# thuml/HashGAN

Hardware: AMD Instinct MI355X
Metric: queries/sec (mAP@R of Q queries vs N-code database, Hamming ranking) (higher is better)
Workload: dtype fp4 (E2M1 0/+-1) x fp4 -> f32 exact distances; u32 xor+popcount elsewhere; f64 AP; 1 GPU; C2: Q=10000 N=1000000 b=64 R=5000 C=10, planted codes; parallelism=1 GPU

## Files before the change

### hashgan_amd/csrc/hg_core.hip

```cpp
#include "hg_ctx.hpp"
#include "hg_host_pack.hpp"

#include <exception>
#include <map>
#include <mutex>
#include <thread>
#include <unistd.h>

thread_local std::string g_err;

int fail(int code, const char* fmt, ...) {
    char buf[512];
    va_list ap;
    va_start(ap, fmt);
    vsnprintf(buf, sizeof buf, fmt, ap);
    va_end(ap);
    g_err = buf;
    return code;
}

const char* const kKernelNames[KI_COUNT] = {"k_hist", "k_hist_reduce", "k_plan", "k_seg_counts", "k_seg_layout", "k_guess",
                                            "k_select", "k_rank_hist", "k_order", "k_rank_fused", "k_match", "k_ap", "k_merge", "k_pack",
                                            "k_real_sample", "k_real_guess", "k_real_select", "k_radix_pass", "k_real_finish", "k_select_mx", "k_rank_cnt", "rccl_allgather", "step_gpu_span", "k_real_rescore"};
void build_shape(int n, ApShape& sh) {
// ... 553 lines not shown
    if (Q < 1 || !host_x || !host_labels) return fail(HG_ERR_ARG, "hg_set_queries_f32: need Q >= 1 and data");
    if (Q > 0x7FFFFFC0ll) return fail(HG_ERR_ARG, "hg_set_queries_f32: Q too large");
    const i64 old_q = c->Q;
    const bool had_q = (c->stage & ST_Q) != 0;
    c->Q = Q;
    if (c->opt.host_pack) {
        const int saved_bpad = c->bpad;
        HG_TRY(pack_on_host(c, host_x, host_labels, Q, c->qc, c->qlab, c->qf, c->dbf_resident ? 1 : 0, &c->qf_resident,
                            bad_codes, bad_labels, c->census_q));
        if (!c->qf_resident) c->bpad = saved_bpad;
    } else {
        HG_TRY(pack_on_device(c, host_x, host_labels, Q, c->qc, c->qlab, c->qf, bad_codes, bad_labels, c->census_q));
        c->qf_resident = true;
    }
    c->stage = ST_DB | ST_Q;
    c->qx_valid = false;
    queries_replaced(c, old_q, had_q);
    return HG_OK;
}

int hg_get_packed(hg_ctx* c, int which, uint32_t* host_codes, uint64_t* host_labels) {
    HG_TRY(need(c, which ? (ST_DB | ST_Q) : ST_DB, "hg_get_packed", "hg_set_database / hg_set_queries"));
    const i64 n = which ? c->Q : c->N;
    DevBuf& cd = which ? c->qc : c->db;
    DevBuf& lb = which ? c->qlab : c->dblab;
    if (host_codes) HG_HIP(hipMemcpyAsync(host_codes, cd.p, (size_t)n * c->NW * 4, hipMemcpyDeviceToHost, c->stream));
    if (host_labels) HG_HIP(hipMemcpyAsync(host_labels, lb.p, (size_t)n * c->LW * 8, hipMemcpyDeviceToHost, c->stream));
    return c->sync();
}

int hg_set_queries(hg_ctx* c, const uint64_t* codes, const uint64_t* labels, int64_t Q) {
// ... 18 lines not shown
    memcpy((char*)qs.pin + cb, labels, lb);
    HG_TRY(c->qc.reserve((size_t)Q * c->NW * 4 + 64 * 4));
    HG_TRY(c->qlab.reserve(lb));
    if (cb + lb <= ((size_t)4 << 20)) {
        const i64 nc = (i64)Q * c->NW, nl = (i64)Q * c->LW * 2;
        hipLaunchKernelGGL(k_copy_in, dim3(grid_for(nc + nl)), dim3(256), 0, c->stream, (const u32*)qs.pin, c->qc.as<u32>(), nc, 2 * W, c->NW,
                           (const u32*)((const char*)qs.pin + cb), c->qlab.as<u32>(), nl);
        HG_TRY(c->check_launch("k_copy_in"));
    } else {
        HG_TRY(upload_codes(c, c->qc, (const uint64_t*)qs.pin, Q, W, c->NW));
        HG_HIP(hipMemcpyAsync(c->qlab.p, (const char*)qs.pin + cb, lb, hipMemcpyHostToDevice, c->stream));
    }
    HG_HIP(hipEventRecord(qs.ev, c->stream));
    qs.used = true;
    c->stage = ST_DB | ST_Q;
    c->qx_valid = false;
    c->qf_resident = false;
    queries_replaced(c, old_q, had_q);
    return HG_OK;
}

extern "C++" int do_match(hg_ctx* c) {
    const Geo& g = c->geo;
    const i64 nKB = (g.R + 255) / 256;
    const i64 blocks = nKB * g.Q;
    if (blocks > 0x7FFFFFFFll) return fail(HG_ERR_ARG, "hg_match: Q*R too large for one launch");
    c->t_begin(KI_MATCH);
    hipLaunchKernelGGL(k_match, dim3((unsigned)blocks), dim3(256), 0, c->stream, c->out_idx.as<u32>(),
                       c->dblab.as<u64>(), c->qlab.as<u64>(), c->mbits.as<u64>(), c->RW, (int)nKB, g);
    c->t_end();
    HG_TRY(c->check_launch("k_match"));
// ... 372 lines not shown
        *value = kind == 0 ? g_host_ns[ph].load() / 1000 : kind == 1 ? g_host_calls[ph].load() : g_host_max_ns[ph].load() / 1000;
    }
    else if (!strcmp(key, "graph_replays")) *value = c->graph_replays;
    else if (!strcmp(key, "cut_beyond_planes")) {
        u32 v = 0;
        if (c->beyond.p) {
            HG_HIP(hipMemcpyAsync(&v, c->beyond.p, 4, hipMemcpyDeviceToHost, c->stream));
            HG_TRY(c->sync());
        }
        *value = v;
    }
    else if (!strcmp(key, "map_async_steps")) *value = c->map_async_steps;
    else if (!strcmp(key, "map_async_redone")) *value = c->map_async_redone;
    else if (!strcmp(key, "map_overlapped_steps")) *value = c->map_overlapped;
    else if (!strcmp(key, "segments")) *value = c->geo.S;
    else if (!strcmp(key, "records_kept")) {
        const Geo& g = c->geo;
        *value = -1;
        if (c->optimistic && c->sl_cnt.p && c->sl_cnt.cap >= (size_t)g.S * g.Qpad * 4) {
            HG_TRY(c->use());
            HG_TRY(c->sync());
            std::vector<u32> h((size_t)g.S * g.Qpad);
            HG_HIP(hipMemcpy(h.data(), c->sl_cnt.p, h.size() * 4, hipMemcpyDeviceToHost));
            i64 total = 0;
            for (int s = 0; s < g.S; ++s) for (int q = 0; q < g.Q; ++q) total += h[(size_t)s * g.Qpad + q];
            *value = total;
        }
    }
    else return fail(HG_ERR_ARG, "hg_get_stat: unknown key '%s'", key);
    return HG_OK;
// ... 45 lines not shown
```

### hashgan_amd/csrc/hg_ctx.hpp

```cpp
#pragma once
#include "hg_kernels.hpp"
#pragma GCC visibility push(default)
#include "../../include/hashgan_amd.h"
#pragma GCC visibility pop

#include <rccl/rccl.h>
#include <atomic>
#include <chrono>
#include <cmath>
#include <cstdarg>
#include <cstdio>
#include <cstdlib>
#include <cstring>
#include <string>
#include <utility>
#include <vector>

using namespace hg;

extern thread_local std::string g_err;
int fail(int code, const char* fmt, ...);

#define HG_HIP(expr)                                                                         \
    do {                                                                                     \
// ... 276 lines not shown
    bool crowd_probed = false;
    i64 crowd_x100 = 0;
    i64 cap_boost = 1;
    i64 real_cap_boost = 1;
    bool leftovers_expected = false;
    bool last_leftovers_inline = false;

    bool want_lists = true;
    i64 bet_runs = 0, bet_fallbacks = 0, bet_requeried = 0;
    i64 rank_leftovers = 0;
    int bet_consecutive_fail = 0;
    int shard_bet_fail = 0;
    hg_ctx* sub = nullptr;
    bool is_sub = false;

    bool dbx_valid = false, qx_valid = false, dbx8_valid = false, dbx3_valid = false, dbx4_valid = false;
    bool hist_pairs = false;
    i64 bet_rebets = 0;
    bool verdict_pending = false, verdict_known = false;
    int verdict_flag = 0;
    void* pin = nullptr;
    size_t pin_cap = 0;
    struct MapSlot {
        void* pin = nullptr; size_t cap = 0; hipEvent_t ev = nullptr;
        bool async = false;
        bool inline_ok = false;
        i64 R = 0, Q = 0;
        unsigned long long q_gen = 0, db_gen = 0;
        std::vector<double> ap; std::vector<int64_t> rel;
    } mslot[2];
    int ms_head = 0, ms_n = 0;
// ... 30 lines not shown
    void* hpk = nullptr;
    size_t hpk_cap = 0;
    bool dbf_resident = false, qf_resident = false;
    RealState real;
    bool real_lists = false;
    i64 shapes_for_R = -1;
    i64 recip_for_R = -1;

    ncclComm_t comm = nullptr;
    int comm_rank = 0, comm_world = 1;

    DevBuf db, dblab, qc, qlab;
    DevBuf dbf, qf;
    DevBuf dbx, qx;
    DevBuf dbx8;
    DevBuf dbx3;
    DevBuf dbx4;
    DevBuf dbfx;
    DevBuf dbfb, xmax2;
    DevBuf shapes, ap_recip;
    DevBuf seglt, segtie;
    DevBuf mbits2;
    DevBuf part;
    DevBuf obuf[2];
    DevBuf beyond;
    DevBuf stage_in, badcnt;
    DevBuf flist;
    DevBuf dbytes;
    DevBuf samp, thr, sortA, sortB, scores, gtab;
    DevBuf sampx;
    DevBuf cntq;
    DevBuf krows;
    DevBuf thr2;
    DevBuf hist2;
    DevBuf gathered[4], scratch[4], comm_tmp, gath_idx, gath_dist;

    template <class F> void for_each_buf(F&& f) {
        for (DevBuf* d : {&db, &dblab, &qc, &qlab, &dbf, &qf}) f(*d, BUF_TABLE);
        for (DevBuf* d : {&dbx, &qx, &dbx8, &dbx3, &dbx4, &dbfx, &dbfb, &xmax2, &shapes, &ap_recip}) f(*d, BUF_DERIVED);
        for (DevBuf* d : {&seglt, &segtie, &mbits2, &part, &obuf[0], &obuf[1], &beyond, &stage_in, &badcnt, &flist, &dbytes, &samp, &thr,
                          &sortA, &sortB, &scores, &gtab, &sampx, &cntq, &krows, &thr2, &hist2, &comm_tmp, &gath_idx, &gath_dist})
            f(*d, BUF_WORK);
        for (DevBuf& d : gathered) f(d, BUF_WORK);
        for (DevBuf& d : scratch) f(d, BUF_WORK);
        for_each_step_buf(f);
        ws_b.for_each_step_buf(f);
    }
    void forget_derived() {
        dbx_valid = qx_valid = dbx8_valid = dbx3_valid = dbx4_valid = dbfx_valid = dbfb_valid = false;
        shapes_for_R = recip_for_R = -1;
        outblk_q = ws_b.outblk_q = -1;
    }

    struct StepGraph {
        hipGraph_t graph = nullptr;
        hipGraphExec_t exec = nullptr;
        unsigned long long epoch = 0, cfg = 0, seen_epoch = 0, seen_cfg = 0;
        i64 R = -1, seen_R = -1;
        int timing = -1, seen_timing = -1;
        StepState left;
        std::vector<Pending> evs;
    } sg;
    unsigned long long cfg_epoch = 1;
    bool capturing = false;
// ... 103 lines not shown
int do_ap_range(hg_ctx* c, i64 q0, i64 nq, const u32* only = nullptr);
inline int do_ap(hg_ctx* c) { return do_ap_range(c, 0, c->geo.Q); }
int ensure_out_block(hg_ctx* c);
int read_plan_flag(hg_ctx* c, int* flag);
int launch_min_topr(hg_ctx* c, const u32* idx_all, const u8* dist_all, i64 n, int G);
hg_ctx* requery_child(hg_ctx* c, i64 nF);
int stage_ap_download(hg_ctx* c, void* dst = nullptr);
int wait_verdict(hg_ctx* c, bool staged, int* flag);
void make_geometry(hg_ctx* c);
Geo hist_geometry(const hg_ctx* c);
int set_R(hg_ctx* c, int64_t R, int G, int rank);
int launch_hist(hg_ctx* c);
int launch_select_valu(hg_ctx* c, int lw, bool optimistic);
int launch_select_dense(hg_ctx* c, int lw);
int ensure_mx_images(hg_ctx* c, bool need_db);
int launch_hist_mx(hg_ctx* c);
int launch_select_mx(hg_ctx* c, int lw, const int* cut);
int launch_select_mx3(hg_ctx* c, int lw, const int* cut);
int launch_select_mx4(hg_ctx* c, int lw, const int* cut);
int preload_valu(); int preload_mx(); int preload_mx1(); int preload_real(); int preload_seq();
void comm_release(hg_ctx* c);

#define HG_DISPATCH_NW(fn, c, ...)                              \
    switch ((c)->NW) {                                          \
        case 1: return fn<1>(c, ##__VA_ARGS__);                 \
        case 2: return fn<2>(c, ##__VA_ARGS__);                 \
        case 3: return fn<3>(c, ##__VA_ARGS__);                 \
        case 4: return fn<4>(c, ##__VA_ARGS__);                 \
        case 5: return fn<5>(c, ##__VA_ARGS__);                 \
        case 6: return fn<6>(c, ##__VA_ARGS__);                 \
// ... 5 lines not shown
```

### hashgan_amd/csrc/hg_hist_i8.hpp

```cpp
#pragma once
#include "hg_kernels.hpp"
#include "hg_hist_mx.hpp"

namespace hg {

typedef int i32x16 __attribute__((ext_vector_type(16)));
typedef __attribute__((address_space(3))) u32 lds_u32;

__device__ __forceinline__ void lds_add_at(const u32 addr, const u32 inc) {
#if defined(__HIP_DEVICE_COMPILE__)
    __hip_atomic_fetch_add((lds_u32*)addr, inc, __ATOMIC_RELAXED, __HIP_MEMORY_SCOPE_WORKGROUP);
#else
    (void)addr; (void)inc;
#endif
}

__device__ __forceinline__ uint4 bits16_to_bytes(const u32 bits, const u32 one, const u32 zero) {
    u32 w[4];
#pragma unroll
    for (int d = 0; d < 4; ++d) {
        u32 v = 0;
#pragma unroll
        for (int i = 0; i < 4; ++i) v |= (((bits >> (4 * d + i)) & 1u) ? one : zero) << (8 * i);
        w[d] = v;
    }
    return uint4{w[0], w[1], w[2], w[3]};
}

static __global__ __launch_bounds__(256) void k_expand_db_i8(const u32* __restrict__ db, uint4* __restrict__ img, i64 N, i64 n16, int NW) {
    const i64 i = (i64)blockIdx.x * 256 + threadIdx.x;
    if (i >= n16 * NW * 2) return;
    const i64 row = i / (NW * 2);
    const int c = (int)(i - row * NW * 2), m = c >> 1, hh = c & 1;
    const u32 word = row < N ? db[row * NW + m] : 0u;
    img[(((row >> 4) * NW + m) * 2 + hh) * 16 + (row & 15)] = bits16_to_bytes((word >> (16 * hh)) & 0xFFFFu, 8u, 0u);
}

constexpr int hist_i8_cols(bool pack16) { return pack16 ? 1 : 2; }

template <int NW, bool PACK16>
__global__ __launch_bounds__(256) __attribute__((amdgpu_waves_per_eu(4, 4)))
void k_hist_i8(const u32* __restrict__ qc, const u8* __restrict__ dbx8, u32* __restrict__ hist, const Geo g) {
    extern __shared__ __attribute__((aligned(16))) u32 hlds[];
    constexpr int QT = 2, WQ = 32 * QT;
    const int lb = logical_block(g.nBlk);
    if (lb < 0) return;
    const int lane = threadIdx.x & 63;
    const int wave = __builtin_amdgcn_readfirstlane(threadIdx.x >> 6);
    const int nQB = g.nQT;
    const int sp = lb / nQB, qb = lb - sp * nQB;
    const int h = lane >> 5, j = lane & 31;
    const int NB = g.NB, b = g.NB - 1;
    const i64 lo0 = (i64)(2 * sp) * g.L, lo1 = lo0 + g.L;
    const i64 len0 = (lo0 + g.L < g.N ? g.L : g.N - lo0);
    const i64 len1 = lo1 >= g.N ? 0 : (lo1 + g.L < g.N ? g.L : g.N - lo1);
    const i64 mylen = h ? len1 : len0;
    const i64 ntile = ((len0 > len1 ? len0 : len1) + 15) / 16;
    const i64 NG = (g.N + 15) >> 4;
    const int stride = g.hist_stride;

    constexpr int NCOL = hist_i8_cols(PACK16);
    u32* col = hlds + wave * NCOL * NB * 32;
    for (int i = lane; i < NCOL * NB * 32; i += 64) col[i] = 0u;

    const int q0w = (qb * WPB + wave) * WQ;
    i32x4 bq[QT][NW];
    i32x16 biasv[QT];
    u32 inc[QT];
#pragma unroll
    for (int t = 0; t < QT; ++t) {
        const int q = q0w + t * 32 + j;
        int pop = 0;
#pragma unroll
        for (int m = 0; m < NW; ++m) {
            const u32 word = q < g.Q ? qc[(i64)q * NW + m] : 0u;
            pop += __builtin_popcount(word);
            const int first = 32 * m + 16 * h;
            const u32 valid = b - first >= 16 ? 0xFFFFu : (b - first <= 0 ? 0u : (1u << (b - first)) - 1u);
            const u32 bits = (word >> (16 * h)) & 0xFFFFu;
            const uint4 neg = bits16_to_bytes(bits & valid, 0xF0u, 0u);
            const uint4 pos = bits16_to_bytes(~bits & valid, 0x10u, 0u);
            bq[t][m] = i32x4{(int)(neg.x | pos.x), (int)(neg.y | pos.y), (int)(neg.z | pos.z), (int)(neg.w | pos.w)};
        }
        u32* c0 = col + (PACK16 ? 0 : t * NB * 32) + j;
        const int base = (int)(u32)(size_t)(lds_u32*)c0 + 128 * pop;
#pragma unroll
        for (int r = 0; r < 16; ++r) biasv[t][r] = base;
        inc[t] = PACK16 ? (t ? 65536u : 1u) : 1u;
    }
    wave_lds_sync();

    const int ah = (j >> 2) & 1;
    const int ar = (j & 3) + 4 * (j >> 3);
    const i64 ag0 = (ah ? lo1 : lo0) >> 4;
    auto chunk = [&](const i64 T, const int m) -> i32x4 {
        i64 G = ag0 + T;
        G = G < NG ? G : NG - 1;
        return *(const i32x4*)(dbx8 + ((((G * NW + m) * 2 + h) * 16 + ar) * 16));
// ... 20 lines not shown
                for (int r = 0; r < 16; ++r)
                    lds_add_at((u32)acc[r], inc[t]);
            } else {
#pragma unroll
                for (int r = 0; r < 16; ++r)
                    if ((i64)r < left) lds_add_at((u32)acc[r], inc[t]);
            }
        }
#pragma unroll
        for (int m = 0; m < NW; ++m) av[m] = an[m];
    }
    wave_lds_sync();
    const int q = q0w + lane;
    if (q < g.Qpad) {
        u32* __restrict__ out = hist + (i64)sp * NB * g.Qpad + q;
        const int dn = g.hcap > 0 && g.hcap < NB ? g.hcap : NB;
        for (int d = 0; d < dn; ++d) {
            const u32 v = PACK16 ? (col[d * 32 + j] >> (16 * h)) & 0xFFFFu : col[(h * NB + d) * 32 + j];
            out[(i64)d * g.Qpad] = v;
        }
    }
}

}
```

### hashgan_amd/csrc/hg_packed_drain.hpp

```cpp
#pragma once
#include "hg_select_mx.hpp"

namespace hg {

constexpr int PK_QCAP = 128;
constexpr int PK_RING = 16;

__device__ __forceinline__ u32 pk_and_or(const u32 x, const u32 k, const u32 y) {
    u32 d;
    asm("v_and_or_b32 %0, %1, %2, %3" : "=v"(d) : "v"(x), "n"(k), "v"(y));
    return d;
}

struct PackedLds {
    int a, abuf;
    int cl, clbuf, labels;
    int qcodes, qlabels;
    int queue;
    int rings;
    int total;
};
template <class P> __host__ __device__ inline PackedLds packed_lds_layout(int NW, int LW) {
    PackedLds l;
    const int WS = P::ws(LW), WROWS = WS * P::ROWS;
// ... 236 lines not shown
                const u8* ring = rings + ring_index(t) * PK_RING;
                *(u64*)(slice(t) + min(f, cap - 8u)) = *(const u64*)(ring + (f & 8u));
            }
        }
    }
};

template <int LW, class P>
struct PackedBlock {
    int sp, qb;
    int h, j;
    int s;
    bool seg_ok;
    i64 lo0, lo1, len0, len1;
    i64 mylen, minlen;
    i64 nwin;
    i64 NG;

    __device__ __forceinline__ PackedBlock(const int lb, const int lane, const Geo& g) {
        constexpr int WROWS = P::ws(LW) * P::ROWS;
        const int nQB = g.nQT;
        sp = lb / nQB;
        qb = lb - sp * nQB;
        h = lane >> 5; j = lane & 31;
        s = 2 * sp + h;
        seg_ok = s < g.S;
        lo0 = (i64)(2 * sp) * g.L; lo1 = lo0 + g.L;
        len0 = (lo0 + g.L < g.N ? g.L : g.N - lo0);
        len1 = lo1 >= g.N ? 0 : (lo1 + g.L < g.N ? g.L : g.N - lo1);
        mylen = h ? len1 : len0;
        minlen = len0 < len1 ? len0 : len1;
        nwin = ((len0 > len1 ? len0 : len1) + WROWS - 1) / WROWS;
        NG = (g.N + P::ROWS - 1) / P::ROWS;
    }
};

}
```

### hashgan_amd/csrc/hg_pairs_mx.hip

```cpp
#include "hg_ctx.hpp"
#include "hg_mx_drain.hpp"
#include "hg_select_mx.hpp"
#include "hg_select_mx3.hpp"
#include "hg_select_mx4.hpp"
#include "hg_hist_mx.hpp"
#include "hg_hist_i8.hpp"

int ensure_mx_images(hg_ctx* c, const bool need_db) {
    const int NW = c->NW, NM = (NW + 1) / 2;
    if (need_db && !c->dbx_valid) {
        const i64 n16 = (c->N + 15) / 16 * 16;
        HG_TRY(c->dbx.reserve((size_t)(n16 > 0 ? n16 : 16) * NM * 32));
        const i64 items = n16 * 2 * NM;
        c->t_begin(KI_PACK);
        if (items) hipLaunchKernelGGL(k_expand_db, dim3(grid_for(items)), dim3(256), 0, c->stream, c->db.as<u32>(),
                                      c->dbx.as<uint4>(), (i64)c->N, n16, NW, NM);
        c->t_end();
        HG_TRY(c->check_launch("k_expand_db"));
        c->dbx_valid = true;
    }
    if (!c->qx_valid) {
        const i64 qpad = ((i64)c->Q + 511) / 512 * 512;
        HG_TRY(c->qx.reserve((size_t)qpad * NM * 32));
        const i64 items = qpad * 2 * NM;
        c->t_begin(KI_PACK);
        hipLaunchKernelGGL(k_expand_queries, dim3(grid_for(items)), dim3(256), 0, c->stream, c->qc.as<u32>(), c->qx.as<uint4>(),
                           (i64)c->Q, qpad, NW, NM);
        c->t_end();
        HG_TRY(c->check_launch("k_expand_queries"));
        c->qx_valid = true;
    }
    return HG_OK;
}


namespace {
template <int NW> int launch_hist_mx_t(hg_ctx* c) {
    HG_TRY(ensure_mx_images(c, true));
    Geo g = c->geo;
    const int nSP = (g.S + 1) / 2;
    const int nQB = (g.Q + 255) / 256;
    g.nQT = nQB;
    g.nUnits = (i64)nSP * nQB;
    g.wpb = WPB;
    g.nBlk = (int)g.nUnits;
    const i64 tiles_per_half = ((g.L + 15) / 16 + g.hist_stride - 1) / g.hist_stride;
    const i64 visited_per_pair = 2 * tiles_per_half * 16;
    const bool pack16 = visited_per_pair < 65536;
    const size_t lds = (size_t)WPB * (pack16 ? 1 : 2) * g.NB * 32 * 4;
// ... 50 lines not shown
template <int NW, int LW> int launch_select_mx4_t(hg_ctx* c, const int* cut) {
    return launch_select_packed<M4Pack>(c, cut, NW, LW, c->dbx4, c->dbx4_valid, k_expand_db4, "k_expand_db4", &k_select_mx4<NW, LW>, "k_select_mx4");
}

template <int NW> int launch_hist_i8_t(hg_ctx* c) {
    if (!c->dbx8_valid) {
        const i64 n16 = (c->N + 15) / 16 * 16;
        HG_TRY(c->dbx8.reserve((size_t)n16 * NW * 32));
        c->t_begin(KI_PACK);
        hipLaunchKernelGGL(k_expand_db_i8, dim3(grid_for(n16 * NW * 2)), dim3(256), 0, c->stream, c->db.as<u32>(), c->dbx8.as<uint4>(),
                           (i64)c->N, n16, NW);
        c->t_end();
        HG_TRY(c->check_launch("k_expand_db_i8"));
        c->dbx8_valid = true;
    }
    Geo g = c->geo;
    const int nSP = (g.S + 1) / 2;
    const int nQB = (g.Q + 255) / 256;
    g.nQT = nQB;
    g.nUnits = (i64)nSP * nQB;
    g.wpb = WPB;
    g.nBlk = (int)g.nUnits;
    const i64 tiles_per_half = ((g.L + 15) / 16 + g.hist_stride - 1) / g.hist_stride;
    const bool pack16 = 2 * tiles_per_half * 16 < 65536;
    const size_t lds = (size_t)WPB * hist_i8_cols(pack16) * g.NB * 32 * 4;
    c->t_begin(KI_HIST);
    if (pack16) {
        if (lds > 64 * 1024)
            HG_HIP(hipFuncSetAttribute(reinterpret_cast<const void*>(&k_hist_i8<NW, true>), hipFuncAttributeMaxDynamicSharedMemorySize, (int)lds));
        hipLaunchKernelGGL((k_hist_i8<NW, true>), dim3(padded_grid(g.nBlk)), dim3(256), lds, c->stream, c->qc.as<u32>(), c->dbx8.as<u8>(),
                           c->hist.as<u32>(), g);
    } else {
        if (lds > 64 * 1024)
            HG_HIP(hipFuncSetAttribute(reinterpret_cast<const void*>(&k_hist_i8<NW, false>), hipFuncAttributeMaxDynamicSharedMemorySize, (int)lds));
        hipLaunchKernelGGL((k_hist_i8<NW, false>), dim3(padded_grid(g.nBlk)), dim3(256), lds, c->stream, c->qc.as<u32>(), c->dbx8.as<u8>(),
                           c->hist.as<u32>(), g);
    }
    c->t_end();
    return c->check_launch("k_hist_i8");
}
}

int launch_hist_mx(hg_ctx* c) {
    if (c->opt.hist_mfma == 2 && c->NW <= 4) {
        switch (c->NW) {
            case 1: return launch_hist_i8_t<1>(c);
            case 2: return launch_hist_i8_t<2>(c);
            case 3: return launch_hist_i8_t<3>(c);
            default: return launch_hist_i8_t<4>(c);
        }
    }
// ... 22 lines not shown
```

### hashgan_amd/csrc/hg_select_mx3.hpp

```cpp
#pragma once
#include "hg_packed_drain.hpp"

namespace hg {

constexpr int M3_QT = 2;
constexpr int M3_ROWS = 48;
#ifndef HG_M3_WS
#define HG_M3_WS 4
#endif
__host__ __device__ constexpr int m3_ws(int LW) { return LW <= 1 ? HG_M3_WS : 2; }
constexpr int M3_WS_MAX = HG_M3_WS > 2 ? HG_M3_WS : 2;
#ifndef HG_M3_WPB
#define HG_M3_WPB 8
#endif
#ifndef HG_M3_FLUSH
#define HG_M3_FLUSH 4
#endif
#ifndef HG_M3_ILV
#define HG_M3_ILV 8
#endif
constexpr int M3_WPB = HG_M3_WPB;

__host__ __device__ constexpr int m3_row(int f, int r) { return r < 7 ? 7 * f + r : r < 14 ? 21 + 7 * f + (r - 7) : 42 + 2 * f + (r - 14); }
__host__ __device__ constexpr int m3_shift(int r) { return r < 7 ? r % 3 : r < 14 ? (r - 7) % 3 : r - 14; }
// ... 82 lines not shown
    constexpr int QT = M3_QT, WQ = 32 * QT;
    constexpr int CB = NW * 4, LB = LW * 8;
    constexpr int M3_WS = m3_ws(LW), M3_WROWS = M3_WS * M3_ROWS;
    const PackedLds L = packed_lds_layout<M3Pack>(NW, LW);

    const int lb = logical_block(g.nBlk);
    if (lb < 0) return;
    const int lane = threadIdx.x & 63;
    const int wave = __builtin_amdgcn_readfirstlane(threadIdx.x >> 6);
    const PackedBlock<LW, M3Pack> blk(lb, lane, g);
    const int h = blk.h, j = blk.j, s = blk.s;
    const bool seg_ok = blk.seg_ok;
    const i64 lo0 = blk.lo0, lo1 = blk.lo1, nwin = blk.nwin, NG = blk.NG;

    const int q0w = (blk.qb * M3_WPB + wave) * WQ;
    {
        u32* qcl = (u32*)(mxlds + L.qcodes + wave * WQ * CB);
        for (int e = lane; e < WQ * NW; e += 64) {
            const i64 q = q0w + e / NW;
            qcl[e] = q < g.Q ? qc[q * NW + (e % NW)] : 0u;
        }
        u64* qll = (u64*)(mxlds + L.qlabels + wave * WQ * LB);
        for (int e = lane; e < WQ * LW; e += 64) {
            const i64 q = q0w + e / LW;
            qll[e] = q < g.Q ? qlab[q * LW + (e % LW)] : 0ull;
        }
    }
    i32x4 bq[QT];
    f32x16 cv[QT];
    u32 K[QT][3];
// ... 80 lines not shown
#undef HG_U
        asm volatile("" : "+v"(w[0]), "+v"(w[1]), "+v"(w[2]));
    };

    int clsel = 0;
    if (nwin > 0) stage_window(0, 0, 0);
    for (i64 win = 0; win < nwin; ++win) {
        const int abuf = (int)(win & 1);
        const int clnext = clsel == 2 ? 0 : clsel + 1;
        asm volatile("s_waitcnt vmcnt(0)" ::: "memory");
        __syncthreads();
        if (win + 1 < nwin) stage_window(win + 1, abuf ^ 1, clnext);
        const u8* sa = mxlds + L.a + abuf * L.abuf;
#pragma unroll
        for (int st = 0; st < M3_WS; ++st) {
            i32x4 af[3];
#pragma unroll
            for (int f = 0; f < 3; ++f) af[f] = *(const i32x4*)(sa + ((st * 3 + f) * 64 + lane) * 16);
            f32x16 acc[QT];
#pragma unroll
            for (int t = 0; t < QT; ++t) acc[t] = cv[t];
            u32 w[QT][3];
#if HG_M3_ILV
#pragma unroll
            for (int t = 0; t < QT; ++t) {
                const i32x8 B = {bq[t].x, bq[t].y, bq[t].z, bq[t].w, 0, 0, 0, 0};
#pragma unroll
                for (int f = 0; f < 3; ++f) {
                    const i32x8 A = {af[f].x, af[f].y, af[f].z, af[f].w, 0, 0, 0, 0};
                    acc[t] = f == 0 ? __builtin_amdgcn_mfma_scale_f32_32x32x64_f8f6f4(A, B, acc[t], 4, 4, 0, scale_a, 0, scale_b)
// ... 25 lines not shown
            for (int t = 0; t < QT; ++t) harvest(acc[t], t, w[t]);
#endif
            const i64 base_row = win * M3_WROWS + st * M3_ROWS;
            if (blk.minlen - base_row < M3_ROWS) {
                const i64 left = blk.mylen - base_row;
                const int la = left < 0 ? 0 : left > 21 ? 21 : (int)left, lb2 = left < 21 ? 0 : left > 42 ? 21 : (int)left - 21;
                const u32 ka = ((1u << la) - 1u) << 6, kb = ((1u << lb2) - 1u) << 6;
                u32 kc = 0;
                for (int c = 0; c < 6; ++c) if (42 + c < left) kc |= 1u << (6 + 7 * (c >> 1) + (c & 1));
#pragma unroll
                for (int t = 0; t < QT; ++t) { w[t][0] &= ka; w[t][1] &= kb; w[t][2] &= kc; }
            }
            if (!(kProbes && (a.probe & 2))) dr.push(w, st, (u32)clsel);
            __builtin_amdgcn_sched_barrier(0);
        }
        if (!(kProbes && (a.probe & 2))) dr.end_window(((win + 1) * M3_WS) % M3Pack::FLUSH == 0);
        clsel = clnext;
    }
    dr.finish();

#pragma unroll
    for (int t = 0; t < QT; ++t) {
        const int q = q0w + t * 32 + j;
        if (seg_ok && q < g.Qpad) {
            const bool live = q < g.Q;
            a.sl_cnt[(i64)s * g.Qpad + q] = live ? (dr.cnt[t] < a.cap ? dr.cnt[t] : a.cap) : 0u;
            if ((dr.cnt[t] > a.cap || far[t]) && live) a.fail[q] = 1u;
        }
    }
}

}
```

### hashgan_amd/csrc/hg_select_mx4.hpp

```cpp
#pragma once
#include "hg_packed_drain.hpp"

namespace hg {

constexpr int M4_QT = 2;
constexpr int M4_ROWS = 32;
#ifndef HG_M4_WS
#define HG_M4_WS 2
#endif
constexpr int M4_WS = HG_M4_WS;
constexpr int M4_WPB = 8;
constexpr int M4_NM = 2;

__host__ __device__ constexpr int m4_row(int f, int r) { return 16 * (r >> 3) + 8 * f + (r & 7); }
__host__ __device__ constexpr int m4_shift(int r) { return r & 7; }
__host__ __device__ inline void m4_place(int rho, int& f, int& r) {
    f = (rho >> 3) & 1;
    r = 8 * (rho >> 4) + (rho & 7);
}

static __global__ __launch_bounds__(256) void k_expand_db4(const u32* __restrict__ db, uint4* __restrict__ dbx, i64 N, i64 n32, int NW) {
    const i64 i = (i64)blockIdx.x * 256 + threadIdx.x;
    if (i >= n32 * 4) return;
    const i64 row = i >> 2;
// ... 48 lines not shown
    constexpr int CB = NW * 4, LB = LW * 8;
    constexpr int WROWS = M4_WS * M4_ROWS;
    constexpr int NM = M4_NM;
    const PackedLds L = packed_lds_layout<M4Pack>(NW, LW);

    const int lb = logical_block(g.nBlk);
    if (lb < 0) return;
    const int lane = threadIdx.x & 63;
    const int wave = __builtin_amdgcn_readfirstlane(threadIdx.x >> 6);
    const PackedBlock<LW, M4Pack> blk(lb, lane, g);
    const int h = blk.h, j = blk.j, s = blk.s;
    const bool seg_ok = blk.seg_ok;
    const i64 lo0 = blk.lo0, lo1 = blk.lo1, nwin = blk.nwin, NG = blk.NG;

    const int q0w = (blk.qb * M4_WPB + wave) * WQ;
    {
        u32* qcl = (u32*)(mxlds + L.qcodes + wave * WQ * CB);
        for (int e = lane; e < WQ * NW; e += 64) {
            const i64 q = q0w + e / NW;
            qcl[e] = q < g.Q ? qc[q * NW + (e % NW)] : 0u;
        }
        u64* qll = (u64*)(mxlds + L.qlabels + wave * WQ * LB);
        for (int e = lane; e < WQ * LW; e += 64) {
            const i64 q = q0w + e / LW;
            qll[e] = q < g.Q ? qlab[q * LW + (e % LW)] : 0ull;
        }
    }
    i32x4 bq[QT][NM];
    f32x16 cv[QT];
    u32 alive[QT];
// ... 83 lines not shown
#undef HG_U
        asm volatile("" : "+v"(w[0]), "+v"(w[1]));
    };

    int clsel = 0;
    if (nwin > 0) stage_window(0, 0, 0);
    for (i64 win = 0; win < nwin; ++win) {
        const int abuf = (int)(win & 1);
        const int clnext = clsel == 2 ? 0 : clsel + 1;
        asm volatile("s_waitcnt vmcnt(0)" ::: "memory");
        __syncthreads();
        if (win + 1 < nwin) stage_window(win + 1, abuf ^ 1, clnext);
        const u8* sa = mxlds + L.a + abuf * L.abuf;
#pragma unroll
        for (int st = 0; st < M4_WS; ++st) {
            u32 w[QT][2];
#if HG_M4_SEQ
#pragma unroll
            for (int t = 0; t < QT; ++t) {
                f32x16 acc = cv[t];
#pragma unroll
                for (int f = 0; f < 2; ++f) {
#pragma unroll
                    for (int m = 0; m < NM; ++m) {
                        const i32x4 af = *(const i32x4*)(sa + (((st * 2 + f) * NM + m) * 64 + lane) * 16);
                        const i32x8 A = {af.x, af.y, af.z, af.w, 0, 0, 0, 0};
                        const i32x8 B = {bq[t][m].x, bq[t][m].y, bq[t][m].z, bq[t][m].w, 0, 0, 0, 0};
                        acc = f == 0 ? __builtin_amdgcn_mfma_scale_f32_32x32x64_f8f6f4(A, B, acc, 4, 4, 0, scale_a, 0, scale_b)
                                     : __builtin_amdgcn_mfma_scale_f32_32x32x64_f8f6f4(A, B, acc, 4, 4, 1, scale_a, 0, scale_b);
                    }
// ... 20 lines not shown
            }
#pragma unroll
            for (int t = 0; t < QT; ++t) harvest(acc[t], t, w[t]);
#endif
            const i64 base_row = win * WROWS + st * M4_ROWS;
            if (blk.minlen - base_row < M4_ROWS) {
                const i64 left = blk.mylen - base_row;
                const int la = left < 0 ? 0 : left > 16 ? 16 : (int)left, lb2 = left < 16 ? 0 : left > 32 ? 16 : (int)left - 16;
                const u32 ka = ((1u << la) - 1u) << 7, kb = ((1u << lb2) - 1u) << 7;
#pragma unroll
                for (int t = 0; t < QT; ++t) { w[t][0] &= ka; w[t][1] &= kb; }
            }
            if (!(kProbes && (a.probe & 2))) dr.push(w, st, (u32)clsel);
            __builtin_amdgcn_sched_barrier(0);
        }
        if (!(kProbes && (a.probe & 2))) dr.end_window(((win + 1) * M4_WS) % M4Pack::FLUSH == 0);
        clsel = clnext;
    }
    dr.finish();

#pragma unroll
    for (int t = 0; t < QT; ++t) {
        const int q = q0w + t * 32 + j;
        if (seg_ok && q < g.Qpad) {
            const bool live = q < g.Q;
            a.sl_cnt[(i64)s * g.Qpad + q] = live ? (dr.cnt[t] < a.cap ? dr.cnt[t] : a.cap) : 0u;
            if ((dr.cnt[t] > a.cap || far[t]) && live) a.fail[q] = 1u;
        }
    }
}

}
```

### hashgan_amd/csrc/hg_seq.hip

```cpp
#include "hg_ctx.hpp"
#include <chrono>
#include "hg_select_mx.hpp"
#include "hg_select_mx3.hpp"
#include "hg_select_mx4.hpp"
#include "hg_hist_mx.hpp"
#include "hg_rank_cnt.hpp"
#include "hg_rank_lean.hpp"
#include "hg_rank_dense.hpp"

constexpr i64 SAMPLE_RATIO = 2;

void make_geometry(hg_ctx* c) {
    Geo& g = c->geo;
    g.Q = (int)c->Q;
    g.nQT = (int)((c->Q + 63) / 64);
    g.Qpad = g.nQT * 64;
    g.NW = c->NW; g.NB = c->NB; g.LW = c->LW;
    g.N = c->N; g.R = c->R; g.idx_base = c->idx_base;
    i64 S = (c->opt.target_units + g.nQT - 1) / g.nQT;
    if (S > c->opt.max_segments) S = c->opt.max_segments;
    const i64 maxS = (c->N + c->opt.min_segment - 1) / c->opt.min_segment;
    if (S > maxS) S = maxS;
    if (S < 1) S = 1;
    i64 L = (c->N + S - 1) / S;
// ... 1328 lines not shown
    c->last_leftovers_inline = false;
    HG_TRY(run_oneshot(c, R, false, true));
    HG_TRY(hg_get_ap(c, host_ap, host_rel));
    if (c->optimistic && c->bet_fallbacks + c->bet_requeried + c->bet_rebets == fails0 && (c->rank_leftovers == left0 || c->last_leftovers_inline) && !c->is_sub) {
        c->map_warm_cfg = c->cfg_epoch; c->map_warm_epoch = g_alloc_epoch; c->map_warm_R = R;
        if (c->opt.step_streams >= 2 && c->own_stream && !c->stream_b) HG_TRY(stream_create(c->device, &c->stream_b));
    } else {
        c->map_warm_R = -1;
    }
    return HG_OK;
}

static int prepare_shared(hg_ctx* c, int64_t R, bool* enqueued) {
    *enqueued = false;
    if (c->opt.select_mfma && !c->qx_valid) { HG_TRY(ensure_mx_images(c, false)); *enqueued = true; }
    const bool recip = c->opt.ap_recip && R <= (1ll << 20);
    if (c->shapes_for_R != R || (recip && c->recip_for_R != R)) {
        HG_TRY(set_R(c, R, 1, 0));
        bool use_recip = false;
        HG_TRY(ensure_ap_tables(c, &use_recip));
        *enqueued = true;
    }
    return HG_OK;
}

static int enqueue_bet_on_b(hg_ctx* c, hg_ctx::MapSlot& m, int64_t R, int stride, bool tail_fork) {
    if (!c->stream_b) HG_TRY(stream_create(c->device, &c->stream_b));
    if (!c->ev_pre) HG_HIP(hipEventCreateWithFlags(&c->ev_pre, hipEventDisableTiming));
    if (!c->ev_fork) HG_HIP(hipEventCreateWithFlags(&c->ev_fork, hipEventDisableTiming));
    if (tail_fork || !c->pre_valid) {
// ... 113 lines not shown
```

Before: 12.20 million queries/s.

## Precompute int8 query image for histogram and skip idle waves in MFMA select

Adds a cached int8 query image with per-query popcounts, built once per query set, so k_hist_i8 loads query fragments instead of expanding bits per block. The histogram LDS clear is limited to the capped distance range. The mx3/mx4 select kernels skip waves whose queries lie entirely past Q and stop stepping past the real segment length, avoiding padded MFMA work. This adds a derived buffer and its validity tracking, and makes the image build part of prepare_shared.

Result: no change. 12.30 million queries/s, median of 6 (+0.8%).

```diff
diff --git a/hashgan_amd/csrc/hg_core.hip b/hashgan_amd/csrc/hg_core.hip
--- a/hashgan_amd/csrc/hg_core.hip
+++ b/hashgan_amd/csrc/hg_core.hip
@@ -591,7 +591,7 @@
         c->qf_resident = true;
     }
     c->stage = ST_DB | ST_Q;
-    c->qx_valid = false;
+    c->qx_valid = c->qx8_valid = false;
     queries_replaced(c, old_q, had_q);
     return HG_OK;
 }
@@ -640,7 +640,7 @@
     HG_HIP(hipEventRecord(qs.ev, c->stream));
     qs.used = true;
     c->stage = ST_DB | ST_Q;
-    c->qx_valid = false;
+    c->qx_valid = c->qx8_valid = false;
     c->qf_resident = false;
     queries_replaced(c, old_q, had_q);
     return HG_OK;
@@ -1043,6 +1043,7 @@
     else if (!strcmp(key, "map_async_redone")) *value = c->map_async_redone;
     else if (!strcmp(key, "map_overlapped_steps")) *value = c->map_overlapped;
     else if (!strcmp(key, "segments")) *value = c->geo.S;
+    else if (!strcmp(key, "segment_rows")) *value = c->geo.L;
     else if (!strcmp(key, "records_kept")) {
         const Geo& g = c->geo;
         *value = -1;
diff --git a/hashgan_amd/csrc/hg_ctx.hpp b/hashgan_amd/csrc/hg_ctx.hpp
--- a/hashgan_amd/csrc/hg_ctx.hpp
+++ b/hashgan_amd/csrc/hg_ctx.hpp
@@ -314,7 +314,7 @@
     hg_ctx* sub = nullptr;
     bool is_sub = false;
 
-    bool dbx_valid = false, qx_valid = false, dbx8_valid = false, dbx3_valid = false, dbx4_valid = false;
+    bool dbx_valid = false, qx_valid = false, qx8_valid = false, dbx8_valid = false, dbx3_valid = false, dbx4_valid = false;
     bool hist_pairs = false;
     i64 bet_rebets = 0;
     bool verdict_pending = false, verdict_known = false;
@@ -375,6 +375,7 @@
     DevBuf dbf, qf;
     DevBuf dbx, qx;
     DevBuf dbx8;
+    DevBuf qx8;
     DevBuf dbx3;
     DevBuf dbx4;
     DevBuf dbfx;
@@ -398,7 +399,7 @@
 
     template <class F> void for_each_buf(F&& f) {
         for (DevBuf* d : {&db, &dblab, &qc, &qlab, &dbf, &qf}) f(*d, BUF_TABLE);
-        for (DevBuf* d : {&dbx, &qx, &dbx8, &dbx3, &dbx4, &dbfx, &dbfb, &xmax2, &shapes, &ap_recip}) f(*d, BUF_DERIVED);
+        for (DevBuf* d : {&dbx, &qx, &dbx8, &qx8, &dbx3, &dbx4, &dbfx, &dbfb, &xmax2, &shapes, &ap_recip}) f(*d, BUF_DERIVED);
         for (DevBuf* d : {&seglt, &segtie, &mbits2, &part, &obuf[0], &obuf[1], &beyond, &stage_in, &badcnt, &flist, &dbytes, &samp, &thr,
                           &sortA, &sortB, &scores, &gtab, &sampx, &cntq, &krows, &thr2, &hist2, &comm_tmp, &gath_idx, &gath_dist})
             f(*d, BUF_WORK);
@@ -408,7 +409,7 @@
         ws_b.for_each_step_buf(f);
     }
     void forget_derived() {
-        dbx_valid = qx_valid = dbx8_valid = dbx3_valid = dbx4_valid = dbfx_valid = dbfb_valid = false;
+        dbx_valid = qx_valid = qx8_valid = dbx8_valid = dbx3_valid = dbx4_valid = dbfx_valid = dbfb_valid = false;
         shapes_for_R = recip_for_R = -1;
         outblk_q = ws_b.outblk_q = -1;
     }
@@ -542,6 +543,7 @@
 int launch_select_valu(hg_ctx* c, int lw, bool optimistic);
 int launch_select_dense(hg_ctx* c, int lw);
 int ensure_mx_images(hg_ctx* c, bool need_db);
+int ensure_hist_i8_queries(hg_ctx* c);
 int launch_hist_mx(hg_ctx* c);
 int launch_select_mx(hg_ctx* c, int lw, const int* cut);
 int launch_select_mx3(hg_ctx* c, int lw, const int* cut);
diff --git a/hashgan_amd/csrc/hg_hist_i8.hpp b/hashgan_amd/csrc/hg_hist_i8.hpp
--- a/hashgan_amd/csrc/hg_hist_i8.hpp
+++ b/hashgan_amd/csrc/hg_hist_i8.hpp
@@ -36,11 +36,35 @@
     img[(((row >> 4) * NW + m) * 2 + hh) * 16 + (row & 15)] = bits16_to_bytes((word >> (16 * hh)) & 0xFFFFu, 8u, 0u);
 }
 
+__host__ __device__ inline i64 hist_i8_qpad(i64 Q) { return (Q + 511) / 512 * 512; }
+__host__ __device__ inline size_t hist_i8_qimg_bytes(i64 Q, int NW) { return (size_t)hist_i8_qpad(Q) * ((size_t)NW * 32 + 4); }
+static __global__ __launch_bounds__(256) void k_expand_queries_i8(const u32* __restrict__ qc, u8* __restrict__ img, i64 Q, i64 qpad, int NW, int b) {
+    const i64 i = (i64)blockIdx.x * 256 + threadIdx.x;
+    if (i >= qpad * NW * 2) return;
+    const i64 q = i / (NW * 2);
+    const int c = (int)(i - q * NW * 2), m = c >> 1, hh = c & 1;
+    const u32 word = q < Q ? qc[q * NW + m] : 0u;
+    const int first = 32 * m + 16 * hh;
+    const u32 valid = b - first >= 16 ? 0xFFFFu : (b - first <= 0 ? 0u : (1u << (b - first)) - 1u);
+    const u32 bits = (word >> (16 * hh)) & 0xFFFFu;
+    const uint4 neg = bits16_to_bytes(bits & valid, 0xF0u, 0u);
+    const uint4 pos = bits16_to_bytes(~bits & valid, 0x10u, 0u);
+    ((uint4*)img)[((q >> 5) * NW + m) * 64 + hh * 32 + (q & 31)] = uint4{neg.x | pos.x, neg.y | pos.y, neg.z | pos.z, neg.w | pos.w};
+    if (c == 0) {
+        int pop = 0;
+        for (int w = 0; w < NW; ++w) pop += __builtin_popcount(q < Q ? qc[q * NW + w] : 0u);
+        ((u32*)(img + (size_t)qpad * NW * 32))[q] = (u32)pop;
+    }
+}
+
 constexpr int hist_i8_cols(bool pack16) { return pack16 ? 1 : 2; }
+#ifndef HG_HIST_QIMG
+#define HG_HIST_QIMG 1
+#endif
 
 template <int NW, bool PACK16>
 __global__ __launch_bounds__(256) __attribute__((amdgpu_waves_per_eu(4, 4)))
-void k_hist_i8(const u32* __restrict__ qc, const u8* __restrict__ dbx8, u32* __restrict__ hist, const Geo g) {
+void k_hist_i8(const u32* __restrict__ qc, const u8* __restrict__ qx8, const u8* __restrict__ dbx8, u32* __restrict__ hist, const Geo g) {
     extern __shared__ __attribute__((aligned(16))) u32 hlds[];
     constexpr int QT = 2, WQ = 32 * QT;
     const int lb = logical_block(g.nBlk);
@@ -50,7 +74,7 @@
     const int nQB = g.nQT;
     const int sp = lb / nQB, qb = lb - sp * nQB;
     const int h = lane >> 5, j = lane & 31;
-    const int NB = g.NB, b = g.NB - 1;
+    const int NB = g.NB;
     const i64 lo0 = (i64)(2 * sp) * g.L, lo1 = lo0 + g.L;
     const i64 len0 = (lo0 + g.L < g.N ? g.L : g.N - lo0);
     const i64 len1 = lo1 >= g.N ? 0 : (lo1 + g.L < g.N ? g.L : g.N - lo1);
@@ -61,7 +85,10 @@
 
     constexpr int NCOL = hist_i8_cols(PACK16);
     u32* col = hlds + wave * NCOL * NB * 32;
-    for (int i = lane; i < NCOL * NB * 32; i += 64) col[i] = 0u;
+    const int dn = g.hcap > 0 && g.hcap < NB ? g.hcap : NB;
+#pragma unroll
+    for (int k = 0; k < NCOL; ++k)
+        for (int i = lane; i < (HG_HIST_QIMG ? dn : NB) * 32; i += 64) col[k * NB * 32 + i] = 0u;
 
     const int q0w = (qb * WPB + wave) * WQ;
     i32x4 bq[QT][NW];
@@ -70,6 +97,12 @@
 #pragma unroll
     for (int t = 0; t < QT; ++t) {
         const int q = q0w + t * 32 + j;
+#if HG_HIST_QIMG
+        const int pop = (int)((const u32*)(qx8 + (size_t)hist_i8_qpad(g.Q) * NW * 32))[q];
+#pragma unroll
+        for (int m = 0; m < NW; ++m) bq[t][m] = *(const i32x4*)(qx8 + (((i64)(q0w / 32 + t) * NW + m) * 64 + lane) * 16);
+#else
+        const int b = NB - 1;
         int pop = 0;
 #pragma unroll
         for (int m = 0; m < NW; ++m) {
@@ -82,6 +115,7 @@
             const uint4 pos = bits16_to_bytes(~bits & valid, 0x10u, 0u);
             bq[t][m] = i32x4{(int)(neg.x | pos.x), (int)(neg.y | pos.y), (int)(neg.z | pos.z), (int)(neg.w | pos.w)};
         }
+#endif
         u32* c0 = col + (PACK16 ? 0 : t * NB * 32) + j;
         const int base = (int)(u32)(size_t)(lds_u32*)c0 + 128 * pop;
 #pragma unroll
@@ -132,7 +166,6 @@
     const int q = q0w + lane;
     if (q < g.Qpad) {
         u32* __restrict__ out = hist + (i64)sp * NB * g.Qpad + q;
-        const int dn = g.hcap > 0 && g.hcap < NB ? g.hcap : NB;
         for (int d = 0; d < dn; ++d) {
             const u32 v = PACK16 ? (col[d * 32 + j] >> (16 * h)) & 0xFFFFu : col[(h * NB + d) * 32 + j];
             out[(i64)d * g.Qpad] = v;
diff --git a/hashgan_amd/csrc/hg_packed_drain.hpp b/hashgan_amd/csrc/hg_packed_drain.hpp
--- a/hashgan_amd/csrc/hg_packed_drain.hpp
+++ b/hashgan_amd/csrc/hg_packed_drain.hpp
@@ -5,6 +5,9 @@
 
 constexpr int PK_QCAP = 128;
 constexpr int PK_RING = 16;
+#ifndef HG_PK_SKIP
+#define HG_PK_SKIP 3
+#endif
 
 __device__ __forceinline__ u32 pk_and_or(const u32 x, const u32 k, const u32 y) {
     u32 d;
@@ -274,6 +277,7 @@
     bool seg_ok;
     i64 lo0, lo1, len0, len1;
     i64 mylen, minlen;
+    int nst;
     i64 nwin;
     i64 NG;
 
@@ -290,7 +294,9 @@
         len1 = lo1 >= g.N ? 0 : (lo1 + g.L < g.N ? g.L : g.N - lo1);
         mylen = h ? len1 : len0;
         minlen = len0 < len1 ? len0 : len1;
-        nwin = ((len0 > len1 ? len0 : len1) + WROWS - 1) / WROWS;
+        const i64 maxlen = len0 > len1 ? len0 : len1;
+        nwin = (maxlen + WROWS - 1) / WROWS;
+        nst = (int)((maxlen + P::ROWS - 1) / P::ROWS);
         NG = (g.N + P::ROWS - 1) / P::ROWS;
     }
 };
diff --git a/hashgan_amd/csrc/hg_pairs_mx.hip b/hashgan_amd/csrc/hg_pairs_mx.hip
--- a/hashgan_amd/csrc/hg_pairs_mx.hip
+++ b/hashgan_amd/csrc/hg_pairs_mx.hip
@@ -33,6 +33,19 @@
     return HG_OK;
 }
 
+
+int ensure_hist_i8_queries(hg_ctx* c) {
+    if (c->qx8_valid || c->opt.hist_mfma != 2 || !c->opt.select_mfma || c->NW > 4 || c->is_sub) return HG_OK;
+    const i64 qpad = hist_i8_qpad(c->Q);
+    HG_TRY(c->qx8.reserve(hist_i8_qimg_bytes(c->Q, c->NW)));
+    c->t_begin(KI_PACK);
+    hipLaunchKernelGGL(k_expand_queries_i8, dim3(grid_for(qpad * c->NW * 2)), dim3(256), 0, c->stream, c->qc.as<u32>(), c->qx8.as<u8>(),
+                       (i64)c->Q, qpad, c->NW, c->NB - 1);
+    c->t_end();
+    HG_TRY(c->check_launch("k_expand_queries_i8"));
+    c->qx8_valid = true;
+    return HG_OK;
+}
 
 namespace {
 template <int NW> int launch_hist_mx_t(hg_ctx* c) {
@@ -113,6 +126,8 @@
         HG_TRY(c->check_launch("k_expand_db_i8"));
         c->dbx8_valid = true;
     }
+    HG_TRY(ensure_hist_i8_queries(c));
+    if (!c->qx8_valid) return fail(HG_ERR_ARG, "k_hist_i8: no query image (hist_mx_applies and ensure_hist_i8_queries disagree)");
     Geo g = c->geo;
     const int nSP = (g.S + 1) / 2;
     const int nQB = (g.Q + 255) / 256;
@@ -127,13 +142,13 @@
     if (pack16) {
         if (lds > 64 * 1024)
             HG_HIP(hipFuncSetAttribute(reinterpret_cast<const void*>(&k_hist_i8<NW, true>), hipFuncAttributeMaxDynamicSharedMemorySize, (int)lds));
-        hipLaunchKernelGGL((k_hist_i8<NW, true>), dim3(padded_grid(g.nBlk)), dim3(256), lds, c->stream, c->qc.as<u32>(), c->dbx8.as<u8>(),
-                           c->hist.as<u32>(), g);
+        hipLaunchKernelGGL((k_hist_i8<NW, true>), dim3(padded_grid(g.nBlk)), dim3(256), lds, c->stream, c->qc.as<u32>(), c->qx8.as<u8>(),
+                           c->dbx8.as<u8>(), c->hist.as<u32>(), g);
     } else {
         if (lds > 64 * 1024)
             HG_HIP(hipFuncSetAttribute(reinterpret_cast<const void*>(&k_hist_i8<NW, false>), hipFuncAttributeMaxDynamicSharedMemorySize, (int)lds));
-        hipLaunchKernelGGL((k_hist_i8<NW, false>), dim3(padded_grid(g.nBlk)), dim3(256), lds, c->stream, c->qc.as<u32>(), c->dbx8.as<u8>(),
-                           c->hist.as<u32>(), g);
+        hipLaunchKernelGGL((k_hist_i8<NW, false>), dim3(padded_grid(g.nBlk)), dim3(256), lds, c->stream, c->qc.as<u32>(), c->qx8.as<u8>(),
+                           c->dbx8.as<u8>(), c->hist.as<u32>(), g);
     }
     c->t_end();
     return c->check_launch("k_hist_i8");
diff --git a/hashgan_amd/csrc/hg_select_mx3.hpp b/hashgan_amd/csrc/hg_select_mx3.hpp
--- a/hashgan_amd/csrc/hg_select_mx3.hpp
+++ b/hashgan_amd/csrc/hg_select_mx3.hpp
@@ -120,6 +120,7 @@
     const i64 lo0 = blk.lo0, lo1 = blk.lo1, nwin = blk.nwin, NG = blk.NG;
 
     const int q0w = (blk.qb * M3_WPB + wave) * WQ;
+    const bool wave_on = !(HG_PK_SKIP & 1) || __builtin_amdgcn_readfirstlane(q0w) < g.Q;
     {
         u32* qcl = (u32*)(mxlds + L.qcodes + wave * WQ * CB);
         for (int e = lane; e < WQ * NW; e += 64) {
@@ -230,6 +231,7 @@
         const u8* sa = mxlds + L.a + abuf * L.abuf;
 #pragma unroll
         for (int st = 0; st < M3_WS; ++st) {
+            if (!wave_on || ((HG_PK_SKIP & 2) && (int)win * M3_WS + st >= blk.nst)) break;
             i32x4 af[3];
 #pragma unroll
             for (int f = 0; f < 3; ++f) af[f] = *(const i32x4*)(sa + ((st * 3 + f) * 64 + lane) * 16);
@@ -285,10 +287,10 @@
             if (!(kProbes && (a.probe & 2))) dr.push(w, st, (u32)clsel);
             __builtin_amdgcn_sched_barrier(0);
         }
-        if (!(kProbes && (a.probe & 2))) dr.end_window(((win + 1) * M3_WS) % M3Pack::FLUSH == 0);
+        if (wave_on && !(kProbes && (a.probe & 2))) dr.end_window(((win + 1) * M3_WS) % M3Pack::FLUSH == 0);
         clsel = clnext;
     }
-    dr.finish();
+    if (wave_on) dr.finish();
 
 #pragma unroll
     for (int t = 0; t < QT; ++t) {
diff --git a/hashgan_amd/csrc/hg_select_mx4.hpp b/hashgan_amd/csrc/hg_select_mx4.hpp
--- a/hashgan_amd/csrc/hg_select_mx4.hpp
+++ b/hashgan_amd/csrc/hg_select_mx4.hpp
@@ -86,6 +86,7 @@
     const i64 lo0 = blk.lo0, lo1 = blk.lo1, nwin = blk.nwin, NG = blk.NG;
 
     const int q0w = (blk.qb * M4_WPB + wave) * WQ;
+    const bool wave_on = !(HG_PK_SKIP & 1) || __builtin_amdgcn_readfirstlane(q0w) < g.Q;
     {
         u32* qcl = (u32*)(mxlds + L.qcodes + wave * WQ * CB);
         for (int e = lane; e < WQ * NW; e += 64) {
@@ -199,6 +200,7 @@
         const u8* sa = mxlds + L.a + abuf * L.abuf;
 #pragma unroll
         for (int st = 0; st < M4_WS; ++st) {
+            if (!wave_on || ((HG_PK_SKIP & 2) && (int)win * M4_WS + st >= blk.nst)) break;
             u32 w[QT][2];
 #if HG_M4_SEQ
 #pragma unroll
@@ -249,10 +251,10 @@
             if (!(kProbes && (a.probe & 2))) dr.push(w, st, (u32)clsel);
             __builtin_amdgcn_sched_barrier(0);
         }
-        if (!(kProbes && (a.probe & 2))) dr.end_window(((win + 1) * M4_WS) % M4Pack::FLUSH == 0);
+        if (wave_on && !(kProbes && (a.probe & 2))) dr.end_window(((win + 1) * M4_WS) % M4Pack::FLUSH == 0);
         clsel = clnext;
     }
-    dr.finish();
+    if (wave_on) dr.finish();
 
 #pragma unroll
     for (int t = 0; t < QT; ++t) {
diff --git a/hashgan_amd/csrc/hg_seq.hip b/hashgan_amd/csrc/hg_seq.hip
--- a/hashgan_amd/csrc/hg_seq.hip
+++ b/hashgan_amd/csrc/hg_seq.hip
@@ -1366,6 +1366,7 @@
 static int prepare_shared(hg_ctx* c, int64_t R, bool* enqueued) {
     *enqueued = false;
     if (c->opt.select_mfma && !c->qx_valid) { HG_TRY(ensure_mx_images(c, false)); *enqueued = true; }
+    if (!c->qx8_valid) { HG_TRY(ensure_hist_i8_queries(c)); if (c->qx8_valid) *enqueued = true; }
     const bool recip = c->opt.ap_recip && R <= (1ll << 20);
     if (c->shapes_for_R != R || (recip && c->recip_for_R != R)) {
         HG_TRY(set_R(c, R, 1, 0));
```
